# souhhcong/RaytracingGPU

Hardware: AMD Instinct MI355X
Metric: Mrays/s, cat mesh 1920x1080 (ms/frame in ms_per_step) (higher is better)
Workload: dtype f32; 1 GPU; cat_1920x1080_spp1_b3; scene=cpu_launcher.cpp walls + cat.obj (3954 tris, 2019-node array BVH), num_rays=1, num_bounce=3, depth_convention=cpu_launcher (b+1 segments), rays_per_frame=16588799, ranks=1, frames_in_flight=2, tiling=8-row tiles interleaved over 1 rank(s), variant=8, device=AMD Radeon Graphics (gfx950:sramecc+:xnack-, 256 CUs)

## Files before the change

### raytracinggpu_amd/csrc/rt_kernels.hip.h

```cpp
#pragma once
#include <hip/hip_runtime.h>
#include <stdint.h>
#include "rt_sincos.h"
#include "rt_div.h"

namespace rtk {

constexpr int kMaxSpheres = 16;
constexpr int kMaxMeshes = 16;
constexpr int kMaxSegments = 16;
constexpr int kBlockThreads = 256;
constexpr int kTileW = 32, kTileH = 8;

struct Sphere {
    float cx, cy, cz, R;
    float R2;
    int obj;
};

struct MeshRec {
    int tri_begin;
    int obj;
};

// ... 140 lines not shown
    decided = true;
    if (r.safe) {
        const float ax = (lo.x - O.x) * r.x, bx = (hi.x - O.x) * r.x;
        const float ay = (lo.y - O.y) * r.y, by = (hi.y - O.y) * r.y;
        const float az = (lo.z - O.z) * r.z, bz = (hi.z - O.z) * r.z;
        const float tn = fmaxf(fmaxf(fminf(ax, bx), fminf(ay, by)), fminf(az, bz));
        const float tf = fminf(fminf(fmaxf(ax, bx), fmaxf(ay, by)), fmaxf(az, bz));
        const float M = fmaxf(fmaxf(fmaxf(fabsf(ax), fabsf(bx)), fmaxf(fabsf(ay), fabsf(by))), fmaxf(fabsf(az), fabsf(bz)));
        const float d = tf - tn;
        const float band = 2.f * (M * kRel + kAbs);
        if (M < kBig) {
            if (d > band) return true;
            if (d < -band) return false;
        }
    }
    decided = false;
    return slab(lo, hi, O, u);
}
__device__ __forceinline__ bool slab_filtered(float4 lo, float4 hi, f3 O, f3 u, const RayInv &r) {
    bool decided;
    return slab_filtered(lo, hi, O, u, r, decided);
}

struct SphereOrigin { f3 OC; float c; };
__device__ __forceinline__ SphereOrigin sphere_origin(const Sphere &s, f3 O) {
    SphereOrigin so;
    so.OC = O - mk(s.cx, s.cy, s.cz);
    so.c = norm2(so.OC) - s.R2;
    return so;
}
__device__ __forceinline__ bool sphere_dir(const Sphere &s, const SphereOrigin &so, f3 O, f3 u, float &t) {
    const float d = dot(u, so.OC);
    const float delta = d * d - so.c;
    if (delta < 0) return false;
    const float sq = rt_sqrtf(delta);
    float b = -d;
    if (__builtin_expect(__ballot(d == 0.f) != 0ull, 0)) {
        if (d == 0.f) b = dot(u, mk(s.cx, s.cy, s.cz) - O);
    }
    const float t1 = b - sq, t2 = b + sq;
    if (t2 < 0) return false;
    t = t1 < 0 ? t2 : t1;
    return true;
}
__device__ __forceinline__ bool sphere_test(const Sphere &s, f3 O, f3 u, float &t) { return sphere_dir(s, sphere_origin(s, O), O, u, t); }

template <bool STATS>
__device__ __forceinline__ bool mesh_intersect(const Scene &sc, f3 O, f3 u, float tri_tmin, float &t_out, f3 &N_out, int &tri_out, Work &wk) {
    float t_min = 1e9f;
    bool any = false;
    int tri_best = 0;
    f3 Nb = mk(0, 0, 0);
    int node = 0;
    const int n_nodes = sc.n_nodes;
    const RayInv ri = ray_inv(u);
    while (node < n_nodes) {
        const float4 lo = sc.node_lo[node];
        const float4 hi = sc.node_hi[node];
        const int hiw = __float_as_int(hi.w);
        const int low = __float_as_int(lo.w);
        if (STATS) wk.box++;
        if (slab_filtered(lo, hi, O, u, ri)) {
            if (STATS) wk.nodes++;
            if (hiw >= 0) {
                if (STATS) wk.tris += (uint32_t)(hiw - low);
                for (int i = low; i < hiw; ++i) {
                    const float4 q0 = sc.tri[3 * i + 0], q1 = sc.tri[3 * i + 1], q2 = sc.tri[3 * i + 2];
                    const f3 A = mk(q0.x, q0.y, q0.z), e1 = mk(q0.w, q1.x, q1.y), e2 = mk(q1.z, q1.w, q2.x);
                    const f3 N = mk(q2.y, q2.z, q2.w);
                    const float det = dot(u, N);
                    if (det == 0) continue;
                    const f3 AO = A - O;
                    const f3 c = cross(AO, u);
                    const float bn = dot(e2, c);
                    const float gn = -dot(e1, c);
                    bool pass = false;
                    if (fabsf(det) > kTiny) {
                        const float rd = __builtin_amdgcn_rcpf(det);
                        const float b = bn * rd, g = gn * rd;
                        const float eb = fabsf(b) * kRel + kAbs, eg = fabsf(g) * kRel + kAbs;
                        if (b < -eb || b > 1.f + eb || g < -eg || g > 1.f + eg) continue;
                        const float sum = b + g;
                        const float es = eb + eg + fabsf(sum) * 0x1p-22f;
                        if (sum > 1.f + es) continue;
                        pass = b >= eb && b <= 1.f - eb && g >= eg && g <= 1.f - eg && sum <= 1.f - es;
                    }
                    if (!pass) {
                        const float beta = bn / det;
                        const float gamma = gn / det;
                        if (!(0 <= beta && beta <= 1) || !(0 <= gamma && gamma <= 1)) continue;
                        if (!(beta + gamma <= 1)) continue;
                    }
                    const float t = dot(AO, N) / det;
                    if (!(t > 0)) continue;
                    if (t > tri_tmin && t < t_min) { t_min = t; Nb = N; any = true; tri_best = i; }
                }
            }
            node = node + 1;
        } else {
            node = (hiw < 0) ? low : node + 1;
        }
    }
    t_out = t_min;
    N_out = Nb;
    tri_out = tri_best;
    return any;
}

__device__ __forceinline__ int mesh_of_tri(const Scene &sc, int tri) {
    int m = 0;
    for (int k = 1; k < sc.n_meshes; ++k) m = (tri >= sc.mesh[k].tri_begin) ? k : m;
    return m;
}
__device__ __forceinline__ int mesh_obj_of_tri(const Scene &sc, int tri) {
    const int mw = mesh_of_tri(sc, tri);
    int mobj = sc.mesh[0].obj;
    for (int k = 1; k < sc.n_meshes; ++k) mobj = (k == mw) ? sc.mesh[k].obj : mobj;
    return mobj;
}
__device__ __forceinline__ bool mesh_beats_sphere(float t_s, int obj_s, float t_m, int obj_m) { return (obj_s > obj_m) ? !(t_s < t_m) : (t_m < t_s); }

template <bool STATS>
__device__ __forceinline__ bool intersect_all(const Scene &sc, f3 O, f3 u, float tri_tmin, f3 &P, f3 &N, int &objectId, Work &wk) {
    float t_min = 1e9f;
    int id_min = -1;
    int sph_min = -1;
    f3 Nmesh = mk(0, 0, 0);
    for (int k = 0; k < sc.n_spheres; ++k) {
        const Sphere &s = sc.sph[k];
        float t;
        if (!sphere_test(s, O, u, t)) continue;
        if (t < t_min) { t_min = t; id_min = s.obj; sph_min = k; }
    }
    if (sc.mesh_slot >= 0 && sc.n_nodes > 0) {
        float t; f3 Nr; int tri;
        if (mesh_intersect<STATS>(sc, O, u, tri_tmin, t, Nr, tri, wk)) {
            const int mobj = mesh_obj_of_tri(sc, tri);
            if (mesh_beats_sphere(t_min, id_min, t, mobj)) { t_min = t; id_min = mobj; sph_min = -1; Nmesh = Nr; }
        }
    }
    P = O + t_min * u;
    objectId = id_min;
    if (id_min < 0) { N = mk(0, 0, 0); return false; }
    if (sph_min >= 0) {
        const Sphere &s = sc.sph[sph_min];
        N = normalize(O + t_min * u - mk(s.cx, s.cy, s.cz));
    } else {
        N = normalize(Nmesh);
    }
    return true;
}

struct Material { float ar, ag, ab; int mirror; float n_in, n_out; };
__device__ __forceinline__ Material material_of(const Scene &sc, int obj) {
    Material m;
    const float4 a = sc.obj_a[obj], b = sc.obj_b[obj];
    const float2 n = sc.obj_n[obj];
    m.ar = b.x; m.ag = b.y; m.ab = b.z; m.mirror = __float_as_int(a.w); m.n_in = n.x; m.n_out = n.y;
    return m;
}
__device__ __forceinline__ f3 sphere_centre_of(const Scene &sc, int obj) { const float4 a = sc.obj_a[obj]; return mk(a.x, a.y, a.z); }

}

#include "rt_shade.hip.h"

namespace rtk {

template <bool STATS>
__device__ __forceinline__ f3 get_color(const Scene &sc, const Frame &fr, f3 O, f3 u, uint32_t hs, float *lstack, float &rays, Work &wk) {
    const f3 L = mk(sc.Lx, sc.Ly, sc.Lz);
    float refr = 1.f;
    uint64_t ids = 0;
    uint32_t diffuse_mask = 0;
    int nseg = 0;
    for (int d = 0; d < fr.segs; ++d) {
        f3 P, N; int id;
        rays += 1.f;
        if (!intersect_all<STATS>(sc, O, u, fr.tri_tmin, P, N, id, wk)) break;
        nseg = d + 1;
        const Material m = material_of(sc, id);
        if (m.mirror) {
            mirror_step(fr.eps, P, N, O, u);
        } else if (m.n_in != m.n_out) {
            refr = refract_step(m, refr, fr.eps, P, N, O, u).refr_after;
        } else {
            const f3 Pa = P + fr.eps * N;
            const f3 sdir = shadow_dir(L, Pa);
            f3 Pp, Np; int ids_;
            rays += 1.f;
            (void)intersect_all<STATS>(sc, Pa, sdir, fr.tri_tmin, Pp, Np, ids_, wk);
            lstack[d * kBlockThreads] = light_hidden(Pa, Pp, L) ? 0.f : direct_term(sc, L, P, N);
            ids |= (uint64_t)(id & 15) << (4 * d);
            diffuse_mask |= 1u << d;
            u = cosine_bounce(N, hs, d);
            O = Pa;
            refr = 1.f;
        }
    }
    f3 ans = mk(0, 0, 0);
    for (int d = nseg - 1; d >= 0; --d) {
        if (diffuse_mask & (1u << d)) {
            const Material m = material_of(sc, (int)((ids >> (4 * d)) & 15));
            ans = fold_segment(ans, lstack[d * kBlockThreads], mk(m.ar, m.ag, m.ab));
        }
    }
    return ans;
}

__device__ __forceinline__ uint32_t wave_sum(uint32_t v) {
#pragma unroll
    for (int o = 32; o > 0; o >>= 1) v += __shfl_down(v, o, 64);
    return v;
}

template <bool STATS>
__global__ __launch_bounds__(kBlockThreads) void render_kernel(const Scene sc, const Frame fr) {
    extern __shared__ __attribute__((aligned(16))) float smem[];
    const int tid = threadIdx.x;
    const int wave = tid >> 6, lane = tid & 63;
    const int px = blockIdx.x * kTileW + wave * 8 + (lane & 7);
    const int lrow = blockIdx.y * kTileH + (lane >> 3);
    const int row = image_row(fr, lrow);
    const bool active = px < fr.W && lrow < fr.n_rows && row < fr.H;
    Work wk;
    float rays = 0.f;
    if (active) {
    float *lstack = smem + tid;

    const f3 C = mk(sc.camx, sc.camy, sc.camz);
    const uint32_t hp = pixel_hash(fr, row, px, fr.seed);
    f3 total = mk(0, 0, 0);
    for (int s = 0; s < fr.spp; ++s) {
        const uint32_t hs = sample_hash(hp, s);
        const f3 u = jitter_dir(fr, pixel_dir(fr, px, row, fr.z), hs);
        const f3 col = get_color<STATS>(sc, fr, C, u, hs, lstack, rays, wk);
        total = total + col;
    }
    const f3 avg = total / (float)fr.spp;
    fr.out[out_index(fr, lrow, px)] = make_float4(avg.x, avg.y, avg.z, rays);
    }
    if (STATS) {
        const uint32_t r = wave_sum((uint32_t)rays), b = wave_sum(wk.box), n = wave_sum(wk.nodes), t = wave_sum(wk.tris);
        if (lane == 0) {
            atomicAdd(&fr.work[0], (unsigned long long)r); atomicAdd(&fr.work[1], (unsigned long long)b);
            atomicAdd(&fr.work[2], (unsigned long long)n); atomicAdd(&fr.work[3], (unsigned long long)t);
        }
    }
}

__device__ __forceinline__ uint32_t tone1(float c) {
    double v = pow((double)c, 1. / 2.2);
    if (255. < v) v = 255.;
    if (!(v == v)) return 0u;
    return (uint32_t)(int)v;
}
__global__ __launch_bounds__(256) void tonemap_kernel(const float4 *__restrict__ rgba, int64_t npix, uint8_t *__restrict__ out) {
    const int64_t q = (int64_t)blockIdx.x * blockDim.x + threadIdx.x;
    const int64_t p0 = q * 4;
    if (p0 >= npix) return;
    uint32_t b[12];
#pragma unroll
    for (int k = 0; k < 4; ++k) {
        float4 c = (p0 + k < npix) ? rgba[p0 + k] : make_float4(0, 0, 0, 0);
        b[3 * k + 0] = tone1(c.x); b[3 * k + 1] = tone1(c.y); b[3 * k + 2] = tone1(c.z);
    }
    if (p0 + 4 <= npix) {
        uint32_t *o = reinterpret_cast<uint32_t *>(out + 3 * p0);
        o[0] = b[0] | (b[1] << 8) | (b[2] << 16) | (b[3] << 24);
        o[1] = b[4] | (b[5] << 8) | (b[6] << 16) | (b[7] << 24);
        o[2] = b[8] | (b[9] << 8) | (b[10] << 16) | (b[11] << 24);
    } else {
        for (int64_t k = 0; p0 + k < npix; ++k)
            for (int ch = 0; ch < 3; ++ch) out[3 * (p0 + k) + ch] = (uint8_t)b[3 * k + ch];
    }
}

__global__ __launch_bounds__(256) void accumulate_kernel(const float4 *__restrict__ frame, float4 *__restrict__ accum, float4 *__restrict__ display,
                                                         uint8_t *__restrict__ rgb8, int64_t npix, int framenumber) {
    const int64_t i = (int64_t)blockIdx.x * blockDim.x + threadIdx.x;
    if (i >= npix) return;
    const float4 f = frame[i];
    float4 a = accum[i];
    a.x += f.x; a.y += f.y; a.z += f.z; a.w += f.w;
    accum[i] = a;
    const float inv = 1.0f / (float)framenumber;
    const float4 d = make_float4(a.x * inv, a.y * inv, a.z * inv, a.w);
    display[i] = d;
    const float c[3] = {d.x, d.y, d.z};
    for (int k = 0; k < 3; ++k) {
        double v = (double)powf(c[k], 1 / 2.2f);
        if (!(v < 255.)) v = 255.;
        rgb8[3 * i + k] = (uint8_t)v;
    }
}

}
```

### raytracinggpu_amd/csrc/rt_wavefront.hip.h

```cpp
#pragma once
#include "rt_kernels.hip.h"
#include "rt_qrows.h"
#include "rt_still.h"
#include <type_traits>

namespace rtk {

constexpr int PF_ALIVE = 1, PF_HASX = 2, PF_HASY = 4;
constexpr int PF_MESHX = 8, PF_MESHY = 16;
constexpr int PF_DEPTH_SHIFT = 5, PF_DEPTH_MASK = 31;
constexpr int PF_RAYS_SHIFT = 10, PF_RAYS_MASK = 63;
constexpr int PF_WINS_SHIFT = 16;
constexpr int PF_XSPHERE = 1 << 26;
constexpr unsigned long long WF_NOHIT = ~0ull;
constexpr int PQ_WIN_SHIFT = 16;
constexpr int PQ_ANYHIT = 1 << 21;
constexpr int PQ_XSPHERE = 1 << 22;
constexpr int PQ_REFR_SHIFT = 23;
constexpr int PQ_TRAV = 1 << 29;
constexpr int PQ_NONCE_SHIFT = 30, PQ_NONCE_MASK = 3;
constexpr int PQ_LIVE_MASK = (int)((unsigned)PQ_TRAV | ((unsigned)PF_DEPTH_MASK << PF_DEPTH_SHIFT) | ((unsigned)PQ_NONCE_MASK << PQ_NONCE_SHIFT));
__device__ __forceinline__ bool wq_live(int w0, int epoch, int nonce) {
    return (w0 & PQ_LIVE_MASK) == (int)((unsigned)PQ_TRAV | (unsigned)epoch << PF_DEPTH_SHIFT | (unsigned)nonce << PQ_NONCE_SHIFT);
}
// ... 448 lines not shown
    }
finished:
    if (dbg_on && lane == 0) {
        st.dbg[6 * wave + 0] = dbg_t0; st.dbg[6 * wave + 1] = __builtin_amdgcn_s_memrealtime();
        st.dbg[6 * wave + 2] = dbg_steps; st.dbg[6 * wave + 3] = dbg_lanes; st.dbg[6 * wave + 4] = dbg_splits; st.dbg[6 * wave + 5] = 0;
        unsigned long long *d2 = st.dbg + 6 * 65536 + 4 * wave;
        d2[0] = cy_box; d2[1] = cy_exp; d2[2] = cy_tri; d2[3] = cy_ref;
    }
#undef WF_STAMP
    wf_flush_work<STATS>(fr, wk);
}

constexpr int kMaxObjects = 16;
constexpr int kSidTextured = 0xfe;
struct TexDesc {
    const uint8_t *texels;
    const float *decode;
    int w, h, ch, filter, wrap, pad;
};
struct TexScene {
    const float2 *uv;
    const TexDesc *desc;
    float4 *ALB;
    int mask;
};
__device__ __forceinline__ f3 tex_texel(const TexDesc &td, int x, int y) {
    const uint8_t *p = td.texels + ((size_t)y * (size_t)td.w + (size_t)x) * (size_t)td.ch;
    return mk(td.decode[p[0]], td.decode[p[1]], td.decode[p[2]]);
}
__device__ __forceinline__ f3 tex_sample(const TexDesc &td, float u, float v) {
    const float W = (float)td.w, H = (float)td.h;
    float fx, fy;
    if (td.filter == 0) {
        const int x = tex_wrap(tex_floor(u * W, fx), td.w, td.wrap), y = tex_wrap(tex_floor((1.f - v) * H, fy), td.h, td.wrap);
        return tex_texel(td, x, y);
    }
    const int x0 = tex_floor(u * W - 0.5f, fx), y0 = tex_floor((1.f - v) * H - 0.5f, fy);
    const int xa = tex_wrap(x0, td.w, td.wrap), xb = tex_wrap(x0 + 1, td.w, td.wrap);
    const int ya = tex_wrap(y0, td.h, td.wrap), yb = tex_wrap(y0 + 1, td.h, td.wrap);
    const f3 t00 = tex_texel(td, xa, ya), t10 = tex_texel(td, xb, ya), t01 = tex_texel(td, xa, yb), t11 = tex_texel(td, xb, yb);
    const float gx = 1.f - fx, gy = 1.f - fy;
    return mk((t00.x * gx + t10.x * fx) * gy + (t01.x * gx + t11.x * fx) * fy,
              (t00.y * gx + t10.y * fx) * gy + (t01.y * gx + t11.y * fx) * fy,
              (t00.z * gx + t10.z * fx) * gy + (t01.z * gx + t11.z * fx) * fy);
}
__device__ __forceinline__ f3 tex_albedo(const Scene &sc, const TexScene &ts, int obj, int tri, const Bary &b, float2 &uv) {
    const float2 ua = ts.uv[3 * tri], ub = ts.uv[3 * tri + 1], uc = ts.uv[3 * tri + 2];
    uv.x = (b.alpha * ua.x + b.beta * ub.x) + b.gamma * uc.x;
    uv.y = (b.alpha * ua.y + b.beta * ub.y) + b.gamma * uc.y;
    const TexDesc td = ts.desc[obj];
    const f3 s = tex_sample(td, uv.x, uv.y);
    const Material m = material_of(sc, obj);
    return mk(m.ar * s.x, m.ag * s.y, m.ab * s.z);
}

#ifdef RT_NO_MARKS
#define ADV_MARK(name) do { } while (0)
#else
#define ADV_MARK(name) do { if constexpr (!LIGHTS && !LENS && !SHUTTER && !SKY && !SAMPLE && !EMIT && !FRESNEL && !GLOSS) asm volatile("rt_mark_adv_" name "_%=:" ::); } while (0)
#endif
struct WfList {
    const unsigned int *items;
    int n;
};
constexpr int kShadeMiss = 0, kShadeDiffuse = 1, kShadeSpecular = 2;
constexpr int SH_SID_SHIFT = 8, SH_REFR_SHIFT = 16, SH_DCH_SHIFT = 22, SH_RAYS_SHIFT = 26;
struct WfShade {
    float4 *rec;
    int kill_x;
};
__device__ __forceinline__ void wf_shade_store(const WfShade &sh, int slot, int kind, f3 O, f3 V, float l0, int sid, int refr_code, int dch, int nrays) {
    const int word = kind | (sid << SH_SID_SHIFT) | (refr_code << SH_REFR_SHIFT) | (dch << SH_DCH_SHIFT) | (int)((unsigned)nrays << SH_RAYS_SHIFT);
    sh.rec[2 * (size_t)slot] = make_float4(O.x, O.y, O.z, V.x);
    sh.rec[2 * (size_t)slot + 1] = make_float4(V.y, V.z, l0, __int_as_float(word));
}
template <class LoadM, class LoadRay>
__device__ __forceinline__ bool wf_x_shadowed(int F, f3 L, LoadM load_m, LoadRay load_ray, unsigned long long &xm) {
    bool shadowed = (F & PQ_XSPHERE) != 0;
    if (!shadowed && (F & PF_MESHX)) {
        const unsigned long long m = load_m();
        xm = m;
        if (m != WF_NOHIT) {
            f3 Oxr, uxr;
            load_ray(Oxr, uxr);
            shadowed = light_hidden(Oxr, uxr, __uint_as_float((unsigned int)(m >> 32)), L);
        }
    }
    return shadowed;
}
constexpr int kMaxLights = 16;
struct WfLights {
    float4 pos[kMaxLights];
    float total;
    int n;
};
__device__ __forceinline__ f3 wf_light_pick(const WfLights &lt, uint32_t hs, int seg) {
    const float x = uniform01(hs, (uint32_t)(seg + 1), 2) * lt.total;
    int k = 0;
    for (int j = 0; j < lt.n; ++j) k += (lt.pos[j].w >= x && lt.pos[j].w > 0.f) ? 0 : 1;
    const float4 p = lt.pos[k < kMaxLights - 1 ? k : kMaxLights - 1];
    return mk(p.x, p.y, p.z);
}
struct WfSoftLights {
    WfLights lt;
    float radius[kMaxLights];
};
__device__ __forceinline__ f3 wf_light_point(const WfSoftLights &sl, uint32_t hs, int seg) {
    const float xk = uniform01(hs, (uint32_t)(seg + 1), 2) * sl.lt.total;
    int k = 0;
    for (int j = 0; j < sl.lt.n; ++j) k += (sl.lt.pos[j].w >= xk && sl.lt.pos[j].w > 0.f) ? 0 : 1;
    k = k < kMaxLights - 1 ? k : kMaxLights - 1;
    const float4 p = sl.lt.pos[k];
    const float rho = sl.radius[k];
    f3 L = mk(p.x, p.y, p.z);
    if (rho > 0.f) {
        const float r1 = uniform01(hs, (1u << 29) + (uint32_t)seg, 0);
        const float r2 = uniform01(hs, (1u << 29) + (uint32_t)seg, 1);
        const float z = 1 - 2 * r1;
        const float s = rt_sqrtf(1 - z * z);
        double sn, cs;
        rt_sincos_2pi(2 * 3.14159265358979323846 * (double)r2, sn, cs);
        const float x = (float)(cs * (double)s);
        const float y = (float)(sn * (double)s);
        L = mk(L.x + rho * x, L.y + rho * y, L.z + rho * z);
    }
    return L;
}
struct WfLens { float radius, focus; };
struct WfGloss {
    unsigned int mask;
    float alpha[kMaxObjects];
};
struct WfShutter {
    float4 light;
    float4 sph[kMaxSpheres];
    float4 obj[kMaxSpheres];
};
__device__ __forceinline__ f3 wf_xyz(float4 v) { return mk(v.x, v.y, v.z); }
using AnimTable = const AnimFrame *__restrict__;
template <unsigned FORM>
__device__ __forceinline__ void wf_advance_path(const Scene &sc, const Frame &fr, const WfState &st, const int i, Work &wk, const TexScene &ts, const AnimFrame *__restrict__ anim,
                                                const WfList &list, const WfShade &sh, const WfLights *__restrict__ lt, const WfSoftLights *__restrict__ sl, const WfLens *__restrict__ ln,
                                                const WfShutter *__restrict__ shu, const WfSky *__restrict__ sky, const WfSkyDist *__restrict__ sd = nullptr,
                                                const WfEmit *__restrict__ em = nullptr, const WfFresnel *__restrict__ fz = nullptr,
                                                const WfGloss *__restrict__ gz = nullptr) {
    constexpr bool STATS = FORM & kFormStats, FIRST = FORM & kFormFirst, TEX = FORM & kFormTex, ANIM = FORM & kFormAnim, LIST = FORM & kFormList;
    constexpr bool FILL = FORM & kFormFill, RESUME = FORM & kFormResume, LENS = FORM & kFormLens, CLOSE = FORM & kFormClose, SHUTTER = FORM & kFormShutter, SKY = FORM & kFormSky;
    constexpr bool SAMPLE = FORM & kFormSkySample;
    constexpr bool EMIT = FORM & kFormEmit;
    constexpr bool FRESNEL = FORM & kFormFresnel;
    constexpr bool GLOSS = FORM & kFormGloss;
    constexpr int LIGHTS = (FORM & kFormSoft) ? 2 : (FORM & kFormLights) ? 1 : 0;
    constexpr bool DEAD_LAST = (FORM & ~kFormStats) == 0u;
    constexpr bool POL_PIXELS = !(TEX && ANIM);
    const float4 kDead = make_float4(0, 0, 0, 0);
    const int rx = st.n_paths + i;
    const int qy = wf_ray_to_slot(st, i), qx = wf_ray_to_slot(st, rx);
    const float4 y1 = (FIRST || RESUME) ? kDead : st.QR[2 * (size_t)qy + 1];
    const int F = __float_as_int(y1.z);
    if (!FIRST && !RESUME && !(F & PF_ALIVE)) {
        if (st.x0 == 1 && !st.m0 && i < st.n_px) st.X0[i] = WF_NOHIT;
        return;
    }
    f3 L = mk(sc.Lx, sc.Ly, sc.Lz);
    int refr_code = (FIRST || RESUME) ? 0 : (F >> PQ_REFR_SHIFT) & 63;
    int d = 0, nrays = 0;
    bool emitY = false, emitX = false, finished = false;
    float x_bound = -__builtin_inff();
    bool x_sky = false;
    bool x_moot = false;
    bool y_dead = false;
    f3 Oy = mk(0, 0, 0), uy = mk(0, 0, 1), Ox = mk(0, 0, 0), ux = mk(0, 0, 1);
    f3 E = mk(0, 0, 0);
    int px, lrow; bool valid;
    int s_rel = 0;
    if (st.n_paths != st.n_px) s_rel = wf_div(i, st.n_px, st.n_px_m);
    float camx = sc.camx, camy = sc.camy, camz = sc.camz, fr_z = fr.z;
    uint32_t fr_seed = fr.seed;
    float4 *fr_out = fr.out;
    int samp = st.samp0 + s_rel;
    bool in_batch = true;
    int af_k = 0;
    if (st.n_batch > 0) {
        const int f = __builtin_amdgcn_readfirstlane(s_rel);
        in_batch = f < st.n_batch;
        const BatchFrame b = st.batch[f & (kMaxBatch - 1)];
        camx = b.camx; camy = b.camy; camz = b.camz;
        fr_z = b.z; fr_seed = b.seed; fr_out = b.out;
        samp = 0;
        if (ANIM) af_k = f & (kMaxBatch - 1);
    }
    const AnimFrame *const af = ANIM ? anim + af_k : nullptr;
    float intensity = sc.intensity;
    if (ANIM) { L = mk(af->Lx, af->Ly, af->Lz); intensity = af->intensity; }
    wf_decode(st, fr, i - s_rel * st.n_px, px, lrow, valid);
    valid = valid && samp < fr.spp && in_batch;
    if (LIST) {
        const unsigned int rec = i < list.n ? list.items[i] : 0u;
        samp = (int)(rec & 63u);
        wf_decode(st, fr, (int)(rec >> 6), px, lrow, valid);
        valid = valid && i < list.n;
    }
    const int row = image_row(fr, lrow);
    float tau = 0.f;
    if constexpr (SHUTTER) {
        tau = shutter_time(sample_hash(pixel_hash(fr, row, px, fr_seed), samp));
        L = shutter_pose(L, wf_xyz(shu->light), tau);
    }
    f3 shO = mk(0, 0, 0), shV = mk(0, 0, 1);
    float sh_l = 0.f;
    int sh_kind = kShadeMiss, sh_sid = 0xff, sh_dch = 0, sh_rays = 0;
    float4 ra = kDead, rb = kDead;
    if (RESUME) {
        if (!valid) { st.QR[2 * (size_t)qy + 1] = kDead; return; }
        if (sh.kill_x) st.QR[2 * (size_t)qx + 1] = kDead;
        const bool nt_rec = (st.policy & kPolRecords) != 0 && st.n_paths == st.n_px;
        ra = pol_load(&sh.rec[2 * (size_t)(i - s_rel * st.n_px)], nt_rec); rb = pol_load(&sh.rec[2 * (size_t)(i - s_rel * st.n_px) + 1], nt_rec);
    }

    if (FIRST) {
        if (!valid) { st.QR[2 * (size_t)qy + 1] = kDead; return; }
        if (st.deadch) st.DCH[i] = 0;
        if (fr.segs <= 0) {
            finished = true;
        } else {
            Oy = mk(camx, camy, camz);
            uy = camera_dir(fr, Oy, fr_z, px, row, sample_hash(pixel_hash(fr, row, px, fr_seed), samp));
            if (LENS) lens_ray(fr, ln->radius, ln->focus, sample_hash(pixel_hash(fr, row, px, fr_seed), samp), Oy, uy);
            emitY = true;
            nrays = 1;
        }
    } else {
        ADV_MARK("closex_begin");
        d = (F >> PF_DEPTH_SHIFT) & PF_DEPTH_MASK;
        nrays = (F >> PF_RAYS_SHIFT) & PF_RAYS_MASK;
        if (RESUME) {
            const int rw = __float_as_int(rb.w);
            sh_kind = rw & 3;
            nrays = (int)((unsigned)rw >> SH_RAYS_SHIFT);
            refr_code = (rw >> SH_REFR_SHIFT) & 63;
            if (st.deadch) st.DCH[i] = (unsigned char)((rw >> SH_DCH_SHIFT) & 15);
        }
        const bool x_close0 = st.x0 != 0 && !st.m0;
        unsigned long long xm = WF_NOHIT;
        if (LIGHTS == 1 && (F & PF_HASX)) L = wf_light_pick(*lt, sample_hash(pixel_hash(fr, row, px, fr_seed), samp), d - 1);
        if constexpr (SAMPLE) x_sky = (F & PF_HASX) && uniform01(sample_hash(pixel_hash(fr, row, px, fr_seed), samp), (uint32_t)d, 3) <= sd->s;
        if constexpr (!EMIT)
        if (LIGHTS == 2 && (F & PF_HASX) && !(SAMPLE && x_sky)) L = wf_light_point(*sl, sample_hash(pixel_hash(fr, row, px, fr_seed), samp), d - 1);
        if constexpr (SAMPLE) {
            if (F & PF_HASX) {
                bool shadowed;
                if (x_sky) shadowed = (F & PQ_XSPHERE) != 0 || ((F & PF_MESHX) != 0 && st.M[rx] != WF_NOHIT);
                else shadowed = wf_x_shadowed(F, L, [&] { return st.M[rx]; }, [&](f3 &Oxr, f3 &uxr) {
                    const float4 x0 = st.QR[2 * (size_t)qx], x1 = st.QR[2 * (size_t)qx + 1];
                    Oxr = mk(x0.x, x0.y, x0.z); uxr = mk(x0.w, x1.x, x1.y);
                }, xm);
                if (shadowed) sd->L3[(size_t)(d - 1) * st.n_paths + i] = make_float4(0.f, 0.f, 0.f, 0.f);
            }
        } else if constexpr (EMIT) {
            if (F & PF_HASX) {
                bool shadowed = (F & PQ_XSPHERE) != 0;
                float4 l4 = make_float4(0.f, 0.f, 0.f, 0.f);
                if (!shadowed && (F & PF_MESHX)) {
                    const unsigned long long m = st.M[rx];
                    if (m != WF_NOHIT) {
                        const float4 x0 = st.QR[2 * (size_t)qx], x1 = st.QR[2 * (size_t)qx + 1];
                        l4 = em->L3[(size_t)(d - 1) * st.n_paths + i];
                        shadowed = light_hidden_far2(mk(x0.x, x0.y, x0.z), mk(x0.w, x1.x, x1.y), __uint_as_float((unsigned int)(m >> 32)), l4.w);
                    }
                }
                if (shadowed) em->L3[(size_t)(d - 1) * st.n_paths + i] = make_float4(0.f, 0.f, 0.f, l4.w);
            }
        } else
        if (!RESUME && (F & PF_HASX)) {
            const bool shadowed = wf_x_shadowed(F, L, [&] {
                const int first = s_rel * st.n_px;
                return !x_close0 ? st.M[rx] : st.x0 == 2 ? st.X0[i - first] : st.M[rx - first];
            }, [&](f3 &Oxr, f3 &uxr) {
                const float4 x0 = st.QR[2 * (size_t)qx], x1 = st.QR[2 * (size_t)qx + 1];
                Oxr = mk(x0.x, x0.y, x0.z); uxr = mk(x0.w, x1.x, x1.y);
            }, xm);
            if (shadowed) st.LS[(size_t)(d - 1) * st.n_paths + i] = 0.f;
        }
        if (!RESUME && x_close0 && st.x0 == 1 && s_rel == 0) st.X0[i] = xm;
        ADV_MARK("closex_end");
        if (!CLOSE && (RESUME || (F & PF_HASY))) {
            ADV_MARK("closey_begin");
            const float4 r0 = RESUME ? ra : st.QR[2 * (size_t)qy];
            f3 O = mk(r0.x, r0.y, r0.z), u = RESUME ? mk(ra.w, rb.x, rb.y) : mk(r0.w, y1.x, y1.y);
            int sid = 0xff;
            float t_min = y1.w;
            int win = ((F >> PQ_WIN_SHIFT) & 31) - 1, tri_win = -1;
            if (RESUME) win = sh_kind == kShadeMiss ? -1 : 0;
            if (!RESUME && (F & PF_MESHY)) {
                const unsigned long long m = st.M[st.m0 ? i - s_rel * st.n_px : i];
                if (m != WF_NOHIT) {
                    const float tm = __uint_as_float((unsigned int)(m >> 32));
                    const int mobj = mesh_obj_of_tri(sc, (int)(unsigned int)m);
                    if (mesh_beats_sphere(t_min, win, tm, mobj)) { t_min = tm; win = mobj; tri_win = (int)(unsigned int)m; }
                }
            }
            if constexpr (EMIT) {
                if (win >= 0 && ((em->mask >> win) & 1u) != 0) {
                    if (d == 0 || !(em->s > 0.f) || st.SID[(size_t)(d - 1) * st.n_paths + i] == 0xff) {
                        const float4 le = em->le[win];
                        E = mk(le.x, le.y, le.z);
                    }
                    win = -1;
                }
            }
            if (win >= 0) {
                const f3 P = O + t_min * u;
                Bary bary{0.f, 0.f, 0.f};
                bool have_bary = false;
                f3 N;
                if (RESUME) N = u;
                else if (ANIM && tri_win < 0) { const float4 c = af->ctr[win]; N = normalize(P - mk(c.x, c.y, c.z)); }
                else if (SHUTTER && tri_win < 0) N = normalize(P - shutter_pose(sphere_centre_of(sc, win), wf_xyz(shu->obj[win]), tau));
                else N = hit_normal(sc, win, tri_win, O, u, P, bary, have_bary);
                const Material m = material_of(sc, win);
                ADV_MARK("closey_end");
                bool cont = false;
                bool fresnel_hit = false;
                if constexpr (FRESNEL) fresnel_hit = ((fz->mask >> win) & 1u) != 0;
                bool gloss_hit = false;
                if constexpr (GLOSS) gloss_hit = ((gz->mask >> win) & 1u) != 0;
                if (gloss_hit) {
                    if constexpr (GLOSS) {
                        gloss_step(fr.eps, gz->alpha[win], P, N, O, u, sample_hash(pixel_hash(fr, row, px, fr_seed), samp), d);
                        cont = true;
                    }
                } else if (!RESUME && m.mirror) {
                    mirror_step(fr.eps, P, N, O, u);
                    cont = true;
                } else if (fresnel_hit) {
                    if constexpr (FRESNEL) {
                        float refr = 1.f;
                        if (refr_code != 0) { const Material mr = material_of(sc, (refr_code >> 1) - 1); refr = (refr_code & 1) ? mr.n_out : mr.n_in; }
                        const Refraction r = fresnel_step(m, refr, fr.eps, P, N, O, u, sample_hash(pixel_hash(fr, row, px, fr_seed), samp), d).r;
                        if (r.crossed) refr_code = (win + 1) << 1 | (r.out2in ? 0 : 1);
                        cont = true;
                    }
                } else if (RESUME && sh_kind == kShadeSpecular) {
                    cont = true;
                } else if (!RESUME && m.n_in != m.n_out) {
                    float refr = 1.f;
                    if (refr_code != 0) { const Material mr = material_of(sc, (refr_code >> 1) - 1); refr = (refr_code & 1) ? mr.n_out : mr.n_in; }
                    const Refraction r = refract_step(m, refr, fr.eps, P, N, O, u);
                    if (r.crossed) refr_code = (win + 1) << 1 | (r.out2in ? 0 : 1);
                    cont = true;
                } else {
                    ADV_MARK("diffuse_begin");
                    const f3 Pa = RESUME ? O : P + fr.eps * N;
                    if (RESUME) {
                        st.LS[i] = rb.z;
                        sid = (__float_as_int(rb.w) >> SH_SID_SHIFT) & 255;
                    } else if constexpr (SAMPLE) {
                        const uint32_t hs = sample_hash(pixel_hash(fr, row, px, fr_seed), samp);
                        x_sky = uniform01(hs, (uint32_t)(d + 1), 3) <= sd->s;
                        f3 l3;
                        Ox = Pa;
                        if (x_sky) {
                            const SkyDraw dr = sky_draw(*sd, hs, d);
                            ux = dr.w;
                            x_bound = __builtin_inff();
                            const float dn = dot(N, dr.w);
                            const float g = sky_weight(*sd, dr.t, dr.m, dr.r, (dn < 0.f) ? 0.f : dn);
                            const f3 Es = sky_radiance(*sky, dr.w);
                            l3 = mk(sd->w_sky * (g * Es.x), sd->w_sky * (g * Es.y), sd->w_sky * (g * Es.z));
                        } else {
                            float nl;
                            L = wf_light_point(*sl, hs, d);
                            ux = shadow_dir(L, Pa, nl);
                            x_bound = wf_anyhit_bound(Pa, nl);
                            const float lv = direct_term(sl->lt.total, L, P, N) * sd->w_light;
                            l3 = mk(lv, lv, lv);
                        }
                        nrays += 1;
                        sd->L3[(size_t)d * st.n_paths + i] = make_float4(l3.x, l3.y, l3.z, 0.f);
                        emitX = true;
                        x_moot = st.anyhit && (__float_as_uint(l3.x) | __float_as_uint(l3.y) | __float_as_uint(l3.z)) == 0u;
                        sid = win;
                        f3 alb = mk(m.ar, m.ag, m.ab);
                        if (TEX && tri_win >= 0 && ((ts.mask >> win) & 1)) {
                            if (!have_bary) bary = tri_bary(sc, tri_win, O, u);
                            float2 uv;
                            alb = tex_albedo(sc, ts, win, tri_win, bary, uv);
                            ts.ALB[(size_t)d * st.n_paths + i] = make_float4(alb.x, alb.y, alb.z, 0.f);
                            sid = kSidTextured;
                        }
                        if (st.deadch) {
                            const int was = st.DCH[i];
                            int now = (was & 8) | (x_sky ? 0 : wf_dead_channels(was & 7, alb, l3.x));
                            if ((now & 7) == 7 && !x_moot) { x_moot = true; now |= 8; }
                            if (now != was) st.DCH[i] = (unsigned char)now;
                        }
                    } else if constexpr (EMIT) {
                        const uint32_t hs = sample_hash(pixel_hash(fr, row, px, fr_seed), samp);
                        const bool x_emit = uniform01(hs, (uint32_t)(d + 1), 3) <= em->s;
                        f3 l3;
                        if (x_emit) {
                            const EmitDraw dr = emit_draw(*em, sc.tri, hs, d);
                            const f3 v = dr.Q - P;
                            const float d2 = norm2(v);
                            const f3 wl = normalize(v);
                            const float dn = dot(N, wl);
                            const float g = emit_weight(*em, dr, wl, d2, (dn < 0.f) ? 0.f : dn);
                            const float4 le = em->le[mesh_obj_of_tri(sc, (int)dr.t)];
                            l3 = mk(em->w_emit * (g * le.x), em->w_emit * (g * le.y), em->w_emit * (g * le.z));
                            L = dr.Q + kEmitKappa * (Pa - dr.Q);
                        } else {
                            L = wf_light_point(*sl, hs, d);
                            const float lv = direct_term(sl->lt.total, L, P, N) * em->w_light;
                            l3 = mk(lv, lv, lv);
                        }
                        float nl;
                        Ox = Pa; ux = shadow_dir(L, Pa, nl);
                        x_bound = wf_anyhit_bound(Pa, nl);
                        nrays += 1;
                        em->L3[(size_t)d * st.n_paths + i] = make_float4(l3.x, l3.y, l3.z, norm2(L - Pa));
                        emitX = true;
                        x_moot = st.anyhit && (__float_as_uint(l3.x) | __float_as_uint(l3.y) | __float_as_uint(l3.z)) == 0u;
                        sid = win;
                        f3 alb = mk(m.ar, m.ag, m.ab);
                        if (TEX && tri_win >= 0 && ((ts.mask >> win) & 1)) {
                            if (!have_bary) bary = tri_bary(sc, tri_win, O, u);
                            float2 uv;
                            alb = tex_albedo(sc, ts, win, tri_win, bary, uv);
                            ts.ALB[(size_t)d * st.n_paths + i] = make_float4(alb.x, alb.y, alb.z, 0.f);
                            sid = kSidTextured;
                        }
                        if (st.deadch) {
                            const int was = st.DCH[i];
                            int now = (was & 8) | (x_emit ? 0 : wf_dead_channels(was & 7, alb, l3.x));
                            if ((now & 7) == 7 && !x_moot) { x_moot = true; now |= 8; }
                            if (now != was) st.DCH[i] = (unsigned char)now;
                        }
                    } else {
                        float nl;
                        if (LIGHTS == 1) { L = wf_light_pick(*lt, sample_hash(pixel_hash(fr, row, px, fr_seed), samp), d); intensity = lt->total; }
                        if (LIGHTS == 2) { L = wf_light_point(*sl, sample_hash(pixel_hash(fr, row, px, fr_seed), samp), d); intensity = sl->lt.total; }
                        Ox = Pa; ux = shadow_dir(L, Pa, nl);
                        x_bound = wf_anyhit_bound(Pa, nl);
                        nrays += 1;
                        const float lvis = (ANIM || LIGHTS) ? direct_term(intensity, L, P, N) : direct_term(sc, L, P, N);
                        st.LS[(size_t)d * st.n_paths + i] = lvis;
                        emitX = true;
                        x_moot = st.anyhit && __float_as_uint(lvis) == 0u;
                        sid = win;
                        f3 alb = mk(m.ar, m.ag, m.ab);
                        if (TEX && tri_win >= 0 && ((ts.mask >> win) & 1)) {
                            if (!have_bary) bary = tri_bary(sc, tri_win, O, u);
                            float2 uv;
                            alb = tex_albedo(sc, ts, win, tri_win, bary, uv);
                            ts.ALB[(size_t)d * st.n_paths + i] = make_float4(alb.x, alb.y, alb.z, 0.f);
                            sid = kSidTextured;
                        }
                        if (st.deadch) {
                            const int was = st.DCH[i];
                            int now = (was & 8) | wf_dead_channels(was & 7, alb, lvis);
                            if ((now & 7) == 7 && !x_moot) {
                                x_moot = true;
                                now |= 8;
                                if (STATS) wk.dead_elided++;
                            }
                            if (now != was) st.DCH[i] = (unsigned char)now;
                            if (FILL) sh_dch = now;
                            if (DEAD_LAST) y_dead = (now & 7) == 7;
                        }
                        if (FILL) { shO = Pa; shV = N; sh_l = lvis; sh_kind = kShadeDiffuse; sh_sid = sid; }
                    }
                    ADV_MARK("diffuse_end");
                    if (d + 1 < fr.segs) {
                        ADV_MARK("bounce_begin");
                        u = cosine_bounce(N, sample_hash(pixel_hash(fr, row, px, fr_seed), samp), d);
                        O = Pa;
                        refr_code = 0;
                        cont = true;
                        ADV_MARK("bounce_end");
                    }
                }
                if (FILL && sid == 0xff) { shO = O; shV = u; sh_kind = kShadeSpecular; }
                if (FILL) sh_rays = nrays;
                if (cont && d + 1 < fr.segs) {
                    emitY = true; Oy = O; uy = u;
                    nrays += 1;
                }
            } else if constexpr (SKY) {
                if (!SAMPLE || d == 0 || st.SID[(size_t)(d - 1) * st.n_paths + i] == 0xff)
                    E = sky_radiance(*sky, u);
            }
            st.SID[(size_t)d * st.n_paths + i] = (unsigned char)sid;
            d = d + 1;
        }
        finished = !(emitX || emitY);
    }

    if (finished) {
        ADV_MARK("fold_begin");
        if (FILL && s_rel == 0)
            wf_shade_store(sh, i, sh_kind, shO, shV, 0.f, 0xff, sh_kind == kShadeSpecular ? refr_code : 0, 0, sh_kind == kShadeMiss ? nrays : sh_rays);
        f3 ans = (SKY || EMIT) ? E : mk(0, 0, 0);
        bool fold_sure = true;
        const int nseg = d < fr.segs ? d : fr.segs;
        for (int k = nseg - 1; k >= 0; --k) {
            const int sid = st.SID[(size_t)k * st.n_paths + i];
            if (sid != 0xff) {
                f3 alb;
                if (TEX && sid == kSidTextured) {
                    const float4 a = ts.ALB[(size_t)k * st.n_paths + i];
                    alb = mk(a.x, a.y, a.z);
                } else {
                    const Material m = material_of(sc, sid);
                    alb = mk(m.ar, m.ag, m.ab);
                }
                if constexpr (SAMPLE) {
                    const float4 l4 = sd->L3[(size_t)k * st.n_paths + i];
                    ans = fold_segment(ans, mk(l4.x, l4.y, l4.z), alb);
                } else if constexpr (EMIT) {
                    const float4 l4 = em->L3[(size_t)k * st.n_paths + i];
                    ans = fold_segment(ans, mk(l4.x, l4.y, l4.z), alb);
                } else {
                const float l = st.LS[(size_t)k * st.n_paths + i];
                ans = fold_segment(ans, l, alb);
                if (STATS && !wf_fold_bounded(ans, l, alb)) fold_sure = false;
                }
            }
        }
        if (STATS && !fold_sure && st.deadch && (st.DCH[i] & 8)) wk.dead_unsure++;
        if (st.samp_out != nullptr) {
            st.samp_out[i] = make_float4(ans.x, ans.y, ans.z, (float)nrays);
        } else {
            float4 t = make_float4(0, 0, 0, 0);
            if (fr.cam_mode == 1) { t.x += ans.x * fr.inv_n; t.y += ans.y * fr.inv_n; t.z += ans.z * fr.inv_n; }
            else { t.x += ans.x; t.y += ans.y; t.z += ans.z; }
            t.w += (float)nrays;
            const float n = fr.cam_mode == 1 ? 1.f : (float)fr.spp;
            pol_store(&fr_out[out_index(fr, lrow, px)], make_float4(t.x / n, t.y / n, t.z / n, t.w), POL_PIXELS && (st.policy & kPolPixels) != 0);
        }
        if (!CLOSE) st.QR[2 * (size_t)qy + 1] = kDead;
        ADV_MARK("fold_end");
        return;
    }

    int flags = PF_ALIVE | (d << PF_DEPTH_SHIFT) | (nrays << PF_RAYS_SHIFT) | (refr_code << PQ_REFR_SHIFT) | (int)((unsigned)st.nonce << PQ_NONCE_SHIFT);
    SphereNear h, hx;
    ADV_MARK("spheres_begin");
    if (ANIM) spheres_near2(sc, af->sph, emitX ? Ox : Oy, uy, emitY, ux, emitX && !x_moot, h, hx);
    else if constexpr (SHUTTER)
        spheres_near2(sc.n_spheres, [&](int k) {
            const Sphere &s0 = sc.sph[k];
            const f3 c = shutter_pose(mk(s0.cx, s0.cy, s0.cz), wf_xyz(shu->sph[k]), tau);
            return Sphere{c.x, c.y, c.z, s0.R, s0.R2, s0.obj};
        }, emitX ? Ox : Oy, uy, emitY, ux, emitX && !x_moot, h, hx);
    else spheres_near2(sc, emitX ? Ox : Oy, uy, emitY, ux, emitX && !x_moot, h, hx);
    ADV_MARK("spheres_end");
    float t_sph = 0.f;
    if (emitX) {
        const float tS = hx.t;
        flags |= PF_HASX;
        if (!x_moot && ((SAMPLE && x_sky) ? hx.obj >= 0 : light_hidden(Ox, ux, tS, L))) flags |= PQ_XSPHERE;
        if (!x_moot && (!(flags & PQ_XSPHERE) || !st.anyhit) && wf_root_test<STATS>(sc, st, rx, Ox, ux, wk)) {
            flags |= PF_MESHX;
            if (STATS) wk.trav_x++;
            const int x_trav = (st.x0 != 0 && st.m0 && (st.x0 == 2 || s_rel != 0)) ? 0 : PQ_TRAV;
            st.QR[2 * (size_t)qx] = make_float4(Ox.x, Ox.y, Ox.z, ux.x);
            st.QR[2 * (size_t)qx + 1] = make_float4(ux.y, ux.z, __int_as_float((int)((unsigned)(x_trav | (st.anyhit ? PQ_ANYHIT : 0) | (d << PF_DEPTH_SHIFT)) | (unsigned)st.nonce << PQ_NONCE_SHIFT)), x_bound);
        }
    }
    if (FILL && s_rel == 0) {
        float l0 = sh_l;
        unsigned long long xw = WF_NOHIT;
        if (emitX && wf_x_shadowed(flags, L, [&] { return st.X0[i]; }, [&](f3 &Oxr, f3 &uxr) { Oxr = Ox; uxr = ux; }, xw)) l0 = 0.f;
        wf_shade_store(sh, i, sh_kind, shO, shV, l0, sh_sid, sh_kind == kShadeSpecular ? refr_code : 0, sh_dch, sh_rays);
    }
    if (emitY) {
        t_sph = h.t;
        flags |= PF_HASY | (((h.obj + 1) & 31) << PQ_WIN_SHIFT);
        bool dead_y = false;
        if constexpr (DEAD_LAST) dead_y = (st.policy & kPolDeadLast) != 0 && y_dead && d == fr.segs - 1 && fr.segs >= 3 && h.obj >= 0;
        if (!(dead_y && !STATS) && wf_root_test<STATS>(sc, st, i, Oy, uy, wk)) {
            flags |= PF_MESHY | PQ_TRAV;
            if (FIRST && st.m0 && s_rel != 0) flags &= ~PQ_TRAV;
            if (STATS) wk.trav_y++;
            if (STATS && dead_y) wk.dead_last++;
        }
    }
    st.QR[2 * (size_t)qy] = make_float4(Oy.x, Oy.y, Oy.z, uy.x);
    st.QR[2 * (size_t)qy + 1] = make_float4(emitY ? uy.y : 0.f, emitY ? uy.z : 0.f, __int_as_float(flags), t_sph);
}

template <class T> __device__ __forceinline__ const T &adv_extra_or(const T &none) { return none; }
template <class T, class E, class... Rest> __device__ __forceinline__ const T &adv_extra_or(const T &none, const E &e, const Rest &... rest) {
    if constexpr (std::is_same_v<T, E>) return e; else return adv_extra_or(none, rest...);
}
template <class T> __device__ __forceinline__ const T *adv_extra() { return nullptr; }
template <class T, class E, class... Rest> __device__ __forceinline__ const T *adv_extra(const E &e, const Rest &... rest) {
    if constexpr (std::is_same_v<T, E>) return &e; else return adv_extra<T>(rest...);
}
template <class T, class... Extra> constexpr bool adv_takes = (std::is_same_v<T, Extra> || ...);
constexpr int adv_waves(unsigned form) { return (form & kFormGloss) ? ((form & kFormTex) ? 7 : 8) : (form & kFormFresnel) ? ((form & kFormTex) ? 7 : 8) : (form & kFormEmit) ? ((form & kFormTex) ? 6 : 7) : (form & kFormSkySample) ? 6 : (form & kFormTex) && (form & kFormSoft) ? 7 : 8; }
template <unsigned FORM, class... Extra>
__global__ __launch_bounds__(256, adv_waves(FORM)) void wf_advance(const Scene sc, const Frame fr, const WfState st, const Extra... extra) {
    static_assert(adv_takes<TexScene, Extra...> == ((FORM & kFormTex) != 0) && adv_takes<AnimTable, Extra...> == ((FORM & kFormAnim) != 0) &&
                  adv_takes<WfList, Extra...> == ((FORM & kFormList) != 0) && adv_takes<WfShade, Extra...> == ((FORM & (kFormFill | kFormResume)) != 0) &&
                  adv_takes<WfLights, Extra...> == ((FORM & kFormLights) != 0) && adv_takes<WfSoftLights, Extra...> == ((FORM & kFormSoft) != 0) &&
                  adv_takes<WfLens, Extra...> == ((FORM & kFormLens) != 0) && adv_takes<WfShutter, Extra...> == ((FORM & kFormShutter) != 0) &&
                  adv_takes<WfSky, Extra...> == ((FORM & kFormSky) != 0) && adv_takes<WfSkyDist, Extra...> == ((FORM & kFormSkySample) != 0) &&
                  adv_takes<WfEmit, Extra...> == ((FORM & kFormEmit) != 0) && adv_takes<WfFresnel, Extra...> == ((FORM & kFormFresnel) != 0) &&
                  adv_takes<WfGloss, Extra...> == ((FORM & kFormGloss) != 0),
                  "a form's extras are the ones its bits name");
    const int i = blockIdx.x * blockDim.x + threadIdx.x;
    Work wk;
    if (i < st.n_paths)
        wf_advance_path<FORM>(sc, fr, st, i, wk, adv_extra_or(TexScene{}, extra...), adv_extra_or<AnimTable>(nullptr, extra...), adv_extra_or(WfList{}, extra...), adv_extra_or(WfShade{}, extra...),
                              adv_extra<WfLights>(extra...), adv_extra<WfSoftLights>(extra...), adv_extra<WfLens>(extra...), adv_extra<WfShutter>(extra...), adv_extra<WfSky>(extra...), adv_extra<WfSkyDist>(extra...),
                              adv_extra<WfEmit>(extra...), adv_extra<WfFresnel>(extra...), adv_extra<WfGloss>(extra...));
    wf_flush_work<(FORM & kFormStats) != 0>(fr, wk);
}

}
```

Baseline: 32760 Mrays/s.

## Hoist global loads early in plain wavefront advance to overlap memory latency

For the plain (no-feature) advance-path forms, mesh-hit records, the dead-channel byte, the ray origin, and the last three fold segments' SID/LS values are loaded at kernel entry instead of at their use sites. Material and sphere data are fetched together, and empty asm statements force the loads to be issued early. The aim is to cut serialized global-memory round trips and hide their latency. The cost is higher register pressure, which may lower occupancy, and a fold path split into a prefetched part and a remainder loop.

```diff
diff --git a/raytracinggpu_amd/csrc/rt_kernels.hip.h b/raytracinggpu_amd/csrc/rt_kernels.hip.h
--- a/raytracinggpu_amd/csrc/rt_kernels.hip.h
+++ b/raytracinggpu_amd/csrc/rt_kernels.hip.h
@@ -316,14 +316,18 @@
 }
 
 struct Material { float ar, ag, ab; int mirror; float n_in, n_out; };
+__device__ __forceinline__ Material material_from(float4 a, float4 b, float2 n) {
+    Material m;
+    m.ar = b.x; m.ag = b.y; m.ab = b.z; m.mirror = __float_as_int(a.w); m.n_in = n.x; m.n_out = n.y;
+    return m;
+}
+__device__ __forceinline__ f3 sphere_centre_from(float4 a) { return mk(a.x, a.y, a.z); }
 __device__ __forceinline__ Material material_of(const Scene &sc, int obj) {
-    Material m;
     const float4 a = sc.obj_a[obj], b = sc.obj_b[obj];
     const float2 n = sc.obj_n[obj];
-    m.ar = b.x; m.ag = b.y; m.ab = b.z; m.mirror = __float_as_int(a.w); m.n_in = n.x; m.n_out = n.y;
-    return m;
-}
-__device__ __forceinline__ f3 sphere_centre_of(const Scene &sc, int obj) { const float4 a = sc.obj_a[obj]; return mk(a.x, a.y, a.z); }
+    return material_from(a, b, n);
+}
+__device__ __forceinline__ f3 sphere_centre_of(const Scene &sc, int obj) { return sphere_centre_from(sc.obj_a[obj]); }
 
 }
 
diff --git a/raytracinggpu_amd/csrc/rt_wavefront.hip.h b/raytracinggpu_amd/csrc/rt_wavefront.hip.h
--- a/raytracinggpu_amd/csrc/rt_wavefront.hip.h
+++ b/raytracinggpu_amd/csrc/rt_wavefront.hip.h
@@ -624,11 +624,14 @@
     constexpr bool GLOSS = FORM & kFormGloss;
     constexpr int LIGHTS = (FORM & kFormSoft) ? 2 : (FORM & kFormLights) ? 1 : 0;
     constexpr bool DEAD_LAST = (FORM & ~kFormStats) == 0u;
+    constexpr bool PLAIN = (FORM & ~(kFormStats | kFormClose)) == 0u;
     constexpr bool POL_PIXELS = !(TEX && ANIM);
     const float4 kDead = make_float4(0, 0, 0, 0);
     const int rx = st.n_paths + i;
     const int qy = wf_ray_to_slot(st, i), qx = wf_ray_to_slot(st, rx);
     const float4 y1 = (FIRST || RESUME) ? kDead : st.QR[2 * (size_t)qy + 1];
+    float4 y0 = kDead;
+    if constexpr (PLAIN && !CLOSE) y0 = st.QR[2 * (size_t)qy];
     const int F = __float_as_int(y1.z);
     if (!FIRST && !RESUME && !(F & PF_ALIVE)) {
         if (st.x0 == 1 && !st.m0 && i < st.n_px) st.X0[i] = WF_NOHIT;
@@ -647,6 +650,29 @@
     int px, lrow; bool valid;
     int s_rel = 0;
     if (st.n_paths != st.n_px) s_rel = wf_div(i, st.n_px, st.n_px_m);
+    constexpr int kFoldRound = 3;
+    unsigned long long pre_ym = WF_NOHIT, pre_xm = WF_NOHIT;
+    int pre_dch = 0;
+    int pre_sid[kFoldRound];
+    float pre_ls[kFoldRound];
+    if constexpr (PLAIN) {
+        if (!CLOSE && (F & (PF_HASY | PF_MESHY)) == (PF_HASY | PF_MESHY)) pre_ym = st.M[st.m0 ? i - s_rel * st.n_px : i];
+        if ((F & (PF_HASX | PQ_XSPHERE | PF_MESHX)) == (PF_HASX | PF_MESHX)) {
+            const int first = s_rel * st.n_px;
+            pre_xm = !(st.x0 != 0 && !st.m0) ? st.M[rx] : st.x0 == 2 ? st.X0[i - first] : st.M[rx - first];
+        }
+        if (!CLOSE && st.deadch) pre_dch = st.DCH[i];
+        if constexpr (CLOSE) {
+            const int dF = (F >> PF_DEPTH_SHIFT) & PF_DEPTH_MASK;
+            const int nsegF = dF < fr.segs ? dF : fr.segs;
+#pragma unroll
+            for (int j = 0; j < kFoldRound; ++j) {
+                const int k = nsegF - 1 - j;
+                pre_sid[j] = 0xff; pre_ls[j] = 0.f;
+                if (k >= 0) { pre_sid[j] = st.SID[(size_t)k * st.n_paths + i]; pre_ls[j] = st.LS[(size_t)k * st.n_paths + i]; }
+            }
+        }
+    }
     float camx = sc.camx, camy = sc.camy, camz = sc.camz, fr_z = fr.z;
     uint32_t fr_seed = fr.seed;
     float4 *fr_out = fr.out;
@@ -743,6 +769,24 @@
                 }
                 if (shadowed) em->L3[(size_t)(d - 1) * st.n_paths + i] = make_float4(0.f, 0.f, 0.f, l4.w);
             }
+        } else if constexpr (PLAIN) {
+            if (F & PF_HASX) {
+                const bool x_readback = x_close0 && fr.segs == 1;
+                const bool shadowed = wf_x_shadowed(F, L, [&] { return pre_xm; }, [&](f3 &Oxr, f3 &uxr) {
+                    if (x_readback) {
+                        const float4 x0 = st.QR[2 * (size_t)qx], x1 = st.QR[2 * (size_t)qx + 1];
+                        Oxr = mk(x0.x, x0.y, x0.z); uxr = mk(x0.w, x1.x, x1.y);
+                    } else {
+                        if constexpr (CLOSE) y0 = st.QR[2 * (size_t)qy];
+                        float nl;
+                        Oxr = mk(y0.x, y0.y, y0.z); uxr = shadow_dir(L, Oxr, nl);
+                    }
+                }, xm);
+                if (shadowed) {
+                    st.LS[(size_t)(d - 1) * st.n_paths + i] = 0.f;
+                    if constexpr (CLOSE) if (d <= fr.segs) pre_ls[0] = 0.f;
+                }
+            }
         } else
         if (!RESUME && (F & PF_HASX)) {
             const bool shadowed = wf_x_shadowed(F, L, [&] {
@@ -758,14 +802,14 @@
         ADV_MARK("closex_end");
         if (!CLOSE && (RESUME || (F & PF_HASY))) {
             ADV_MARK("closey_begin");
-            const float4 r0 = RESUME ? ra : st.QR[2 * (size_t)qy];
+            const float4 r0 = RESUME ? ra : PLAIN ? y0 : st.QR[2 * (size_t)qy];
             f3 O = mk(r0.x, r0.y, r0.z), u = RESUME ? mk(ra.w, rb.x, rb.y) : mk(r0.w, y1.x, y1.y);
             int sid = 0xff;
             float t_min = y1.w;
             int win = ((F >> PQ_WIN_SHIFT) & 31) - 1, tri_win = -1;
             if (RESUME) win = sh_kind == kShadeMiss ? -1 : 0;
             if (!RESUME && (F & PF_MESHY)) {
-                const unsigned long long m = st.M[st.m0 ? i - s_rel * st.n_px : i];
+                const unsigned long long m = PLAIN ? pre_ym : st.M[st.m0 ? i - s_rel * st.n_px : i];
                 if (m != WF_NOHIT) {
                     const float tm = __uint_as_float((unsigned int)(m >> 32));
                     const int mobj = mesh_obj_of_tri(sc, (int)(unsigned int)m);
@@ -786,11 +830,19 @@
                 Bary bary{0.f, 0.f, 0.f};
                 bool have_bary = false;
                 f3 N;
+                Material m_plain{};
                 if (RESUME) N = u;
                 else if (ANIM && tri_win < 0) { const float4 c = af->ctr[win]; N = normalize(P - mk(c.x, c.y, c.z)); }
                 else if (SHUTTER && tri_win < 0) N = normalize(P - shutter_pose(sphere_centre_of(sc, win), wf_xyz(shu->obj[win]), tau));
+                else if constexpr (PLAIN) {
+                    const float4 oa = sc.obj_a[win], ob = sc.obj_b[win];
+                    const float2 on = sc.obj_n[win];
+                    N = tri_win >= 0 ? hit_normal(sc, win, tri_win, O, u, P, bary, have_bary) : normalize(P - sphere_centre_from(oa));
+                    asm volatile("" :: "v"(oa.w), "v"(ob.x), "v"(ob.y), "v"(ob.z), "v"(on.x), "v"(on.y));
+                    m_plain = material_from(oa, ob, on);
+                }
                 else N = hit_normal(sc, win, tri_win, O, u, P, bary, have_bary);
-                const Material m = material_of(sc, win);
+                const Material m = PLAIN ? m_plain : material_of(sc, win);
                 ADV_MARK("closey_end");
                 bool cont = false;
                 bool fresnel_hit = false;
@@ -913,6 +965,7 @@
                         if (LIGHTS == 1) { L = wf_light_pick(*lt, sample_hash(pixel_hash(fr, row, px, fr_seed), samp), d); intensity = lt->total; }
                         if (LIGHTS == 2) { L = wf_light_point(*sl, sample_hash(pixel_hash(fr, row, px, fr_seed), samp), d); intensity = sl->lt.total; }
                         Ox = Pa; ux = shadow_dir(L, Pa, nl);
+                        if constexpr (PLAIN) Oy = Pa;
                         x_bound = wf_anyhit_bound(Pa, nl);
                         nrays += 1;
                         const float lvis = (ANIM || LIGHTS) ? direct_term(intensity, L, P, N) : direct_term(sc, L, P, N);
@@ -929,7 +982,7 @@
                             sid = kSidTextured;
                         }
                         if (st.deadch) {
-                            const int was = st.DCH[i];
+                            const int was = PLAIN ? pre_dch : st.DCH[i];
                             int now = (was & 8) | wf_dead_channels(was & 7, alb, lvis);
                             if ((now & 7) == 7 && !x_moot) {
                                 x_moot = true;
@@ -975,7 +1028,27 @@
         f3 ans = (SKY || EMIT) ? E : mk(0, 0, 0);
         bool fold_sure = true;
         const int nseg = d < fr.segs ? d : fr.segs;
-        for (int k = nseg - 1; k >= 0; --k) {
+        if constexpr (PLAIN && CLOSE) {
+            f3 pre_alb[kFoldRound];
+#pragma unroll
+            for (int j = 0; j < kFoldRound; ++j) {
+                const float4 b = sc.obj_b[pre_sid[j] != 0xff ? pre_sid[j] : 0];
+                pre_alb[j] = mk(b.x, b.y, b.z);
+            }
+            static_assert(kFoldRound == 3, "the statement below names every albedo");
+            asm volatile("" :: "v"(pre_alb[0].x), "v"(pre_alb[1].x), "v"(pre_alb[2].x));
+#pragma unroll
+            for (int j = 0; j < kFoldRound; ++j) {
+                const int sid = pre_sid[j];
+                if (sid != 0xff) {
+                    const f3 alb = pre_alb[j];
+                    const float l = pre_ls[j];
+                    ans = fold_segment(ans, l, alb);
+                    if (STATS && !wf_fold_bounded(ans, l, alb)) fold_sure = false;
+                }
+            }
+        }
+        for (int k = nseg - 1 - ((PLAIN && CLOSE) ? kFoldRound : 0); k >= 0; --k) {
             const int sid = st.SID[(size_t)k * st.n_paths + i];
             if (sid != 0xff) {
                 f3 alb;
```

After: 33410 Mrays/s, median of 6. 1.02x the previous value.
